# lasgroup/Model-based-policy-optimizers

Hardware: NVIDIA B200
Metric: iCEM model-rollout transitions/sec (pop x horizon x problems x CEM iterations) (higher is better)
Workload: dtype f32

## Files before the change

### model-based-policy-optimizers_b200/csrc/icem_kernels.cuh

```cuda
#pragma once
#include <cuda_runtime.h>

#include "noise.cuh"
#include "pendulum.cuh"
#include "select.cuh"
#include "systems.cuh"

namespace mbpo {

template <int MATH, bool SMALL = false, typename ActFn>
__device__ __forceinline__ float rollout_return_th(const PendulumConsts& pc, float th0, float w0, int H, ActFn act) {
  float acc = 0.0f;
  float th = th0, w = w0;
#pragma unroll 2
  for (int t = 0; t < H; ++t) {
    float r;
    if (MATH == MBPO_MATH_REFERENCE) pendulum_step_ref_th<SMALL>(pc, th, w, act(t), r);
    else pendulum_step_theta<SMALL>(pc, th, w, act(t), r);
    acc = __fadd_rn(acc, r);
  }
  return __fdiv_rn(acc, static_cast<float>(H));
}

template <int MATH, bool SMALL = false, typename ActFn>
__device__ __forceinline__ float rollout_return(const PendulumConsts& pc, float c0, float s0, float w0, int H,
                                                ActFn act) {
  return rollout_return_th<MATH, SMALL>(pc, atan2_bounded(s0, c0), w0, H, act);
}

template <int MATH>
__device__ __forceinline__ void rollout_return2(const PendulumConsts& pc, float th0, float w0, int H,
                                                const float* __restrict__ row_a, const float* __restrict__ row_b,
                                                float& ret_a, float& ret_b) {
  f32x2_t acc = splat2(0.0f), th = splat2(th0), w = splat2(w0);
#pragma unroll 1
  for (int t = 0; t < H; ++t) {
    f32x2_t neg_r;
    if (MATH == MBPO_MATH_REFERENCE) pendulum_step_ref_th2(pc, th, w, pack2(row_a[t], row_b[t]), neg_r);
    else pendulum_step_theta2(pc, th, w, pack2(row_a[t], row_b[t]), neg_r);
    acc = sub2(acc, neg_r);
  }
  float acc_a, acc_b;
  unpack2(acc, acc_a, acc_b);
  ret_a = __fdiv_rn(acc_a, static_cast<float>(H));
  ret_b = __fdiv_rn(acc_b, static_cast<float>(H));
}

__device__ __forceinline__ float summarize_particles(float ret, int P, int summarize) {
  if (summarize == MBPO_SUMMARIZE_MAX || P == 1) return ret;
  float acc = 0.0f;
  for (int p = 0; p < P; ++p) acc = __fadd_rn(acc, ret);
  return __fdiv_rn(acc, static_cast<float>(P));
}

struct PlanArgs {
  int B, N, Np, K, P, S, H;
  int warm_start, summarize;
  float init_std, alpha, one_minus_alpha, u_min, u_max;
  MbpoPendulumParams sys;
  MbpoGeneralSystemParams gsys;
  float scale[MBPO_MAX_FREQ];
  const float* x0;
  const uint32_t* key_in;
  const float* best_seq_in;
  float* best_seq_out;
  float* best_value_out;
  uint32_t* key_out;
  MbpoIcemTrace trace;
  int zero_value_precomputed;
};

constexpr int PLAN_THREADS = 256;

template <int HT>
struct PlanSmem {
  static constexpr int HS = HT | 1;
  static size_t bytes(int N, int Np, int K, int H_rt = 0) {
    const int H = HT ? HT : H_rt;
    const int hs = H | 1;
    size_t words = static_cast<size_t>(N + 1) * hs
                   + (N + Np)
                   + 2 * (N + 1)
                   + 3 * H
                   + 2 * K
                   + select_scratch_words(K, N + Np)
                   + 8
                   + (HT ? 0 : static_cast<size_t>(PLAN_THREADS) * hs);
    return words * 4;
  }
};

template <int HT>
struct PlanCtaSmem {
  float* act;
  uint32_t* skey;
  uint32_t* flat;
  float* mean;
  float* std_;
  float* best_seq;
  int* elite_idx;
  int* sel_idx;
  uint32_t* sel_scratch;
  float* best_value;
  uint32_t* carry;
  uint32_t* state_key;
  float* stage;
  __device__ __forceinline__ PlanCtaSmem(uint32_t* base, int N, int Np, int K, int H_rt = 0) {
    const int H = HT ? HT : H_rt;
    const int HS = H | 1;
    act = reinterpret_cast<float*>(base);
    skey = base + static_cast<size_t>(N + 1) * HS;
    flat = skey + (N + Np);
    mean = reinterpret_cast<float*>(flat + 2 * (N + 1));
    std_ = mean + H;
    best_seq = std_ + H;
    elite_idx = reinterpret_cast<int*>(best_seq + H);
    sel_idx = elite_idx + K;
    sel_scratch = reinterpret_cast<uint32_t*>(sel_idx + K);
    best_value = reinterpret_cast<float*>(sel_scratch + select_scratch_words(K, N + Np));
    carry = reinterpret_cast<uint32_t*>(best_value + 1);
    state_key = carry + 2;
    stage = reinterpret_cast<float*>(state_key + 5);
  }
};

template <int HT, int PRNG, int MATH, int THREADS>
__device__ __forceinline__ void plan_problem(const PlanArgs& a, const PlanCtaSmem<HT>& sm, const PendulumConsts& pc,
                                             const RefitScalars& rs, const float* prev_best, Key2 key_in,
                                             Key2& key_new, float x_th, float x_w, int slot, int slots,
                                             const TwiddleTable* tw = nullptr) {
  const int H = HT ? HT : a.H;
  const int HS = H | 1;
  const int N = a.N, M = a.N + a.Np, K = a.K;
  const int tid = threadIdx.x;
  float* act = sm.act;
  uint32_t* skey = sm.skey;
  uint32_t* flat = sm.flat;
  float* mean = sm.mean;
  float* std_ = sm.std_;
  float* best_seq = sm.best_seq;

  float m0 = 0.0f;
  if (tid < H && a.warm_start) m0 = prev_best[tid + 1 < H ? tid + 1 : H - 1];
  __syncthreads();
  if (tid < H) {
    mean[tid] = m0;
    std_[tid] = a.init_std;
    best_seq[tid] = m0;
  }
  if (tid < HS) act[static_cast<size_t>(N) * HS + tid] = 0.0f;
  if (tid == 0) {
    *sm.best_value = __int_as_float(0xFF800000);
    Key2 k_opt;
    split2<PRNG>(key_in, k_opt, key_new);
    sm.carry[0] = k_opt.k0;
    sm.carry[1] = k_opt.k1;
  }
  __syncthreads();

  for (int it = 0; it < a.S; ++it) {
    const size_t tslot = static_cast<size_t>(it) * slots + slot;
    Key2 ck{sm.carry[0], sm.carry[1]}, sampling_rng, particles_rng;
    split2<PRNG>(ck, sampling_rng, particles_rng);
    if (PRNG == MBPO_PRNG_LEGACY) {
      for (int j = tid; j < N + 1; j += THREADS) {
        uint32_t y0 = static_cast<uint32_t>(j), y1 = static_cast<uint32_t>(N + 1 + j);
        threefry2x32(sampling_rng.k0, sampling_rng.k1, y0, y1);
        flat[j] = y0;
        flat[N + 1 + j] = y1;
      }
    }
    __syncthreads();
    if (tid == 0) {
      Key2 nk;
      if (PRNG == MBPO_PRNG_LEGACY) { nk.k0 = flat[0]; nk.k1 = flat[1]; }
      else nk = split_at<1>(sampling_rng, static_cast<uint32_t>(N + 1), 0u);
      sm.carry[0] = nk.k0; sm.carry[1] = nk.k1;
    }

    const int jobs = (it == 0 && !a.zero_value_precomputed) ? N + 1 : N;
    if (it == 0 && a.zero_value_precomputed && tid == THREADS - 1) {
      const uint32_t zk = total_order_key(a.best_value_out[slot]);
      for (int j = N; j < M; ++j) skey[j] = zk;
    }
    for (int n0 = tid; n0 < jobs; n0 += 2 * THREADS) {
      const int n1 = n0 + THREADS;
#pragma unroll 1
      for (int h = 0; h < 2; ++h) {
        const int n = h ? n1 : n0;
        if (n >= N) continue;
        Key2 skey_n;
        if (PRNG == MBPO_PRNG_LEGACY) { skey_n.k0 = flat[2 * (n + 1)]; skey_n.k1 = flat[2 * (n + 1) + 1]; }
        else skey_n = split_at<1>(sampling_rng, static_cast<uint32_t>(N + 1), static_cast<uint32_t>(n + 1));
        const Key2 dim_key = split1<PRNG>(skey_n);
        float* row = act + static_cast<size_t>(n) * HS;
        auto emit = [&](int t, float y) {
          const float v = __fadd_rn(mean[t], __fmul_rn(y, std_[t]));
          row[t] = fminf(fmaxf(v, a.u_min), a.u_max);
        };
        if constexpr (HT != 0) colored_noise_row<HT, PRNG>(dim_key, a.scale, row, nullptr, emit);
        else colored_noise_row_rt<PRNG>(H, dim_key, a.scale, *tw, sm.stage + static_cast<size_t>(tid) * HS, nullptr, emit);
      }
      const int r0 = n0 < N ? n0 : N, r1 = n1 < N ? n1 : N;
      float ret0, ret1;
      rollout_return2<MATH>(pc, x_th, x_w, H, act + static_cast<size_t>(r0) * HS, act + static_cast<size_t>(r1) * HS,
                            ret0, ret1);
#pragma unroll
      for (int h = 0; h < 2; ++h) {
        const int n = h ? n1 : n0;
        const float val = summarize_particles(h ? ret1 : ret0, a.P, a.summarize);
        if (n < N) {
          skey[n] = total_order_key(val);
          if (a.trace.values) a.trace.values[tslot * M + n] = val;
          if (a.trace.actions) {
            const float* row = act + static_cast<size_t>(n) * HS;
            float* dst = a.trace.actions + (tslot * M + n) * H;
            for (int t = 0; t < H; ++t) dst[t] = row[t];
          }
        } else if (n == N && it == 0) {
          const uint32_t zk = total_order_key(val);
          for (int j = N; j < M; ++j) skey[j] = zk;
        }
      }
    }
    __syncthreads();
    if (a.trace.values || a.trace.actions) {
      const uint32_t zk = skey[N];
      const float zv = __uint_as_float((zk & 0x80000000u) ? (zk & 0x7FFFFFFFu) : ~zk);
      for (int j = N + tid; j < M; j += THREADS) {
        if (a.trace.values) a.trace.values[tslot * M + j] = zv;
        if (a.trace.actions) {
          float* dst = a.trace.actions + (tslot * M + j) * H;
          for (int t = 0; t < H; ++t) dst[t] = 0.0f;
        }
      }
    }

    cta_select_refit<THREADS>(rs, skey, sm.elite_idx, sm.sel_idx, sm.sel_scratch,
                              [&](int i, int d) { return i < N ? act[static_cast<size_t>(i) * HS + d] : 0.0f; },
                              mean, std_, best_seq, sm.best_value);
    if (a.trace.elite_idx)
      for (int e = tid; e < K; e += THREADS) a.trace.elite_idx[tslot * K + e] = sm.elite_idx[e];
    for (int d = tid; d < H; d += THREADS) {
      if (a.trace.mean) a.trace.mean[tslot * H + d] = mean[d];
      if (a.trace.std) a.trace.std[tslot * H + d] = std_[d];
    }
    if (a.trace.best_value && tid == 0) a.trace.best_value[tslot] = *sm.best_value;
    __syncthreads();
  }
}

template <int MATH>
__global__ void zero_row_value_kernel(const MbpoPendulumParams sys, int H, int P, int summarize,
                                      const float* __restrict__ x0, int B, float* __restrict__ out) {
  const int b = blockIdx.x * blockDim.x + threadIdx.x;
  if (b >= B) return;
  const PendulumConsts pc(sys);
  const float ret = rollout_return<MATH, true>(pc, x0[3 * b], x0[3 * b + 1], x0[3 * b + 2], H,
                                               [](int) { return 0.0f; });
  out[b] = summarize_particles(ret, P, summarize);
}

template <int HT, int PRNG, int MATH, int THREADS>
__device__ __forceinline__ void plan_kernel_body(const PlanArgs& a, const TwiddleTable* tw) {
  extern __shared__ __align__(16) uint32_t smem_u32[];
  const int H = HT ? HT : a.H;
  const PlanCtaSmem<HT> sm(smem_u32, a.N, a.Np, a.K, H);
  const int tid = threadIdx.x;
  const PendulumConsts pc(a.sys);
  RefitScalars rs;
  rs.M = a.N + a.Np; rs.K = a.K; rs.D = H; rs.alpha = a.alpha; rs.one_minus_alpha = a.one_minus_alpha;

  for (int b = blockIdx.x; b < a.B; b += gridDim.x) {
    const float x_c = a.x0[3 * b], x_s = a.x0[3 * b + 1], x_w = a.x0[3 * b + 2];
    Key2 k_in{a.key_in[2 * b], a.key_in[2 * b + 1]}, k_new;
    plan_problem<HT, PRNG, MATH, THREADS>(a, sm, pc, rs, a.best_seq_in + static_cast<size_t>(b) * H, k_in, k_new,
                                          atan2_bounded(x_s, x_c), x_w, b, a.B, tw);
    if (tid < H) a.best_seq_out[static_cast<size_t>(b) * H + tid] = sm.best_seq[tid];
    if (tid == 0) {
      a.best_value_out[b] = *sm.best_value;
      a.key_out[2 * b] = k_new.k0;
      a.key_out[2 * b + 1] = k_new.k1;
    }
    __syncthreads();
  }
}

template <int H, int PRNG, int MATH, int THREADS, int MINB>
__global__ void __launch_bounds__(THREADS, MINB) icem_plan_pendulum_kernel(const __grid_constant__ PlanArgs a) {
  plan_kernel_body<H, PRNG, MATH, THREADS>(a, nullptr);
}

template <int PRNG, int MATH>
__global__ void __launch_bounds__(PLAN_THREADS, 1)
    icem_plan_pendulum_rt_kernel(const __grid_constant__ PlanArgs a, const __grid_constant__ TwiddleTable tw) {
  plan_kernel_body<0, PRNG, MATH, PLAN_THREADS>(a, &tw);
}

struct MpcArgs {
  int T;
  float* states_out;
  float* rewards_out;
  float* actions_out;
};

template <int HT, int PRNG, int MATH, int THREADS>
__device__ __forceinline__ void mpc_kernel_body(const PlanArgs& a, const MpcArgs& m, const TwiddleTable* tw) {
  extern __shared__ __align__(16) uint32_t smem_u32[];
  const int H = HT ? HT : a.H;
  const PlanCtaSmem<HT> sm(smem_u32, a.N, a.Np, a.K, H);
  __shared__ float xs[4];
  const int tid = threadIdx.x;
  const PendulumConsts pc(a.sys);
  RefitScalars rs;
  rs.M = a.N + a.Np; rs.K = a.K; rs.D = H; rs.alpha = a.alpha; rs.one_minus_alpha = a.one_minus_alpha;

  for (int b = blockIdx.x; b < a.B; b += gridDim.x) {
    if (tid < H) sm.best_seq[tid] = a.best_seq_in[static_cast<size_t>(b) * H + tid];
    if (tid < 3) xs[tid] = a.x0[3 * b + tid];
    if (tid == 0) { sm.state_key[0] = a.key_in[2 * b]; sm.state_key[1] = a.key_in[2 * b + 1]; }
    __syncthreads();
    for (int t = 0; t < m.T; ++t) {
      const float x_c = xs[0], x_s = xs[1], x_w = xs[2];
      Key2 k_in{sm.state_key[0], sm.state_key[1]}, k_new;
      plan_problem<HT, PRNG, MATH, THREADS>(a, sm, pc, rs, sm.best_seq, k_in, k_new, atan2_bounded(x_s, x_c), x_w, 0,
                                            1, tw);
      if (tid == 0) {
        sm.state_key[0] = k_new.k0; sm.state_key[1] = k_new.k1;
        const float u = sm.best_seq[0];
        float c = x_c, s = x_s, w = x_w, r;
        if (MATH == MBPO_MATH_REFERENCE) {
          pendulum_step_ref(pc, c, s, w, u, r);
        } else {
          float th = atan2_bounded(s, c);
          pendulum_step_theta(pc, th, w, u, r);
          sincos_bounded(th, s, c);
        }
        xs[0] = c; xs[1] = s; xs[2] = w;
        const size_t o = static_cast<size_t>(t) * a.B + b;
        if (m.states_out) { m.states_out[o * 3] = c; m.states_out[o * 3 + 1] = s; m.states_out[o * 3 + 2] = w; }
        if (m.rewards_out) m.rewards_out[o] = r;
        if (m.actions_out) m.actions_out[o] = u;
      }
      __syncthreads();
    }
    if (tid < H) a.best_seq_out[static_cast<size_t>(b) * H + tid] = sm.best_seq[tid];
    if (tid == 0) {
      a.best_value_out ? (void)(a.best_value_out[b] = *sm.best_value) : (void)0;
      a.key_out[2 * b] = sm.state_key[0];
      a.key_out[2 * b + 1] = sm.state_key[1];
    }
    __syncthreads();
  }
}

template <int H, int PRNG, int MATH, int THREADS, int MINB>
__global__ void __launch_bounds__(THREADS, MINB)
    icem_mpc_pendulum_kernel(const __grid_constant__ PlanArgs a, const __grid_constant__ MpcArgs m) {
  mpc_kernel_body<H, PRNG, MATH, THREADS>(a, m, nullptr);
}

template <int PRNG, int MATH>
__global__ void __launch_bounds__(PLAN_THREADS, 1)
    icem_mpc_pendulum_rt_kernel(const __grid_constant__ PlanArgs a, const __grid_constant__ MpcArgs m,
                                const __grid_constant__ TwiddleTable tw) {
  mpc_kernel_body<0, PRNG, MATH, PLAN_THREADS>(a, m, &tw);
}

template <int H, int A>
struct GenPlanSmem {
  static constexpr int RS = (H * A) | 1;
  static size_t bytes(int N, int Np, int K) {
    const size_t words = static_cast<size_t>(N + 1) * RS + (N + Np) + 3 * H * A + 2 * K +
                         select_scratch_words(K, N + Np) + 8;
    return words * 4;
  }
};

template <class Sys, int H, int PRNG>
__global__ void __launch_bounds__(256, 1) icem_plan_general_kernel(const __grid_constant__ PlanArgs a) {
  constexpr int A = Sys::A, X = Sys::X, D = H * A, RS = GenPlanSmem<H, A>::RS, THREADS = 256;
  extern __shared__ __align__(16) uint32_t smem_u32[];
  const int N = a.N, M = a.N + a.Np, K = a.K;
  float* act = reinterpret_cast<float*>(smem_u32);
  uint32_t* skey = smem_u32 + static_cast<size_t>(N + 1) * RS;
  float* mean = reinterpret_cast<float*>(skey + M);
  float* std_ = mean + D;
  float* best_seq = std_ + D;
  int* elite_idx = reinterpret_cast<int*>(best_seq + D);
  int* sel_idx = elite_idx + K;
  uint32_t* scratch = reinterpret_cast<uint32_t*>(sel_idx + K);
  float* best_value = reinterpret_cast<float*>(scratch + select_scratch_words(K, M));
  uint32_t* carry = reinterpret_cast<uint32_t*>(best_value + 1);
  const int tid = threadIdx.x;
  const Sys sys(a.gsys);
  RefitScalars rs;
  rs.M = M; rs.K = K; rs.D = D; rs.alpha = a.alpha; rs.one_minus_alpha = a.one_minus_alpha;
  auto elem = [&](int i, int d) { return i < N ? act[static_cast<size_t>(i) * RS + (d % A) * H + d / A] : 0.0f; };

  for (int b = blockIdx.x; b < a.B; b += gridDim.x) {
    float s0[X];
#pragma unroll
    for (int k = 0; k < X; ++k) s0[k] = a.x0[static_cast<size_t>(b) * X + k];
    const float* prev = a.best_seq_in + static_cast<size_t>(b) * D;
    for (int d = tid; d < D; d += THREADS) {
      float m = 0.0f;
      if (a.warm_start) m = prev[(d + A < D) ? d + A : (D - A + d % A)];
      mean[d] = m;
      std_[d] = a.init_std;
      best_seq[d] = m;
    }
    for (int d = tid; d < RS; d += THREADS) act[static_cast<size_t>(N) * RS + d] = 0.0f;
    Key2 k_new{0u, 0u};
    if (tid == 0) {
      *best_value = __int_as_float(0xFF800000);
      Key2 k_opt;
      split2<PRNG>(Key2{a.key_in[2 * b], a.key_in[2 * b + 1]}, k_opt, k_new);
      carry[0] = k_opt.k0;
      carry[1] = k_opt.k1;
    }
    __syncthreads();
    float zero_value = 0.0f;

    for (int it = 0; it < a.S; ++it) {
      const size_t tslot = static_cast<size_t>(it) * a.B + b;
      Key2 ck{carry[0], carry[1]}, sampling_rng, particles_rng;
      split2<PRNG>(ck, sampling_rng, particles_rng);
      __syncthreads();
      if (tid == 0) {
        const Key2 nk = split_at<PRNG>(sampling_rng, static_cast<uint32_t>(N + 1), 0u);
        carry[0] = nk.k0;
        carry[1] = nk.k1;
      }
      const int jobs = Sys::KEYED ? M : ((it == 0) ? N + 1 : N);
      for (int n = tid; n < jobs; n += THREADS) {
        float* row = act + static_cast<size_t>(n < N ? n : N) * RS;
        if (n < N) {
          const Key2 sk = split_at<PRNG>(sampling_rng, static_cast<uint32_t>(N + 1), static_cast<uint32_t>(n + 1));
#pragma unroll 1
          for (int ad = 0; ad < A; ++ad) {
            const Key2 dk = split_at<PRNG>(sk, static_cast<uint32_t>(A), static_cast<uint32_t>(ad));
            float* dim = row + ad * H;
            colored_noise_row<H, PRNG>(dk, a.scale, dim, nullptr, [&](int t, float y) {
              const float v = __fadd_rn(mean[t * A + ad], __fmul_rn(y, std_[t * A + ad]));
              dim[t] = fminf(fmaxf(v, a.u_min), a.u_max);
            });
          }
        }
        float val;
        auto roll = [&](Key2 key) {
          float s[X];
#pragma unroll
          for (int k = 0; k < X; ++k) s[k] = s0[k];
          float acc = 0.0f;
          for (int t = 0; t < H; ++t) acc = __fadd_rn(acc, sys.template step<PRNG>(s, row + t, H, key));
          return __fdiv_rn(acc, static_cast<float>(H));
        };
        if (!Sys::KEYED) {
          const float ret = roll(Key2{0u, 0u});
          if (a.summarize == MBPO_SUMMARIZE_MAX || a.P == 1) {
            val = ret;
          } else {
            float acc = 0.0f;
            for (int p = 0; p < a.P; ++p) acc = __fadd_rn(acc, ret);
            val = __fdiv_rn(acc, static_cast<float>(a.P));
          }
        } else {
          const Key2 pkey = split_at<PRNG>(particles_rng, static_cast<uint32_t>(M), static_cast<uint32_t>(n));
          float acc = 0.0f, mx = 0.0f;
          for (int p = 0; p < a.P; ++p) {
            const float ret = roll(split_at<PRNG>(pkey, static_cast<uint32_t>(a.P), static_cast<uint32_t>(p)));
            acc = __fadd_rn(acc, ret);
            mx = (p == 0) ? ret : fmaxf(mx, ret);
          }
          val = (a.summarize == MBPO_SUMMARIZE_MAX) ? mx : __fdiv_rn(acc, static_cast<float>(a.P));
        }
        if (n < N || Sys::KEYED) {
          skey[n] = total_order_key(val);
          if (a.trace.values) a.trace.values[tslot * M + n] = val;
        } else {
          zero_value = val;
          for (int j = N; j < M; ++j) skey[j] = total_order_key(val);
        }
        if (a.trace.actions) {
          float* dst = a.trace.actions + (tslot * M + n) * D;
          for (int d = 0; d < D; ++d) dst[d] = (n < N) ? row[(d % A) * H + d / A] : 0.0f;
        }
      }
      __syncthreads();
      if (!Sys::KEYED && (a.trace.values || a.trace.actions)) {
        const float zv = value_of_key(skey[N]);
        for (int j = N + tid; j < M; j += THREADS) {
          if (a.trace.values) a.trace.values[tslot * M + j] = zv;
          if (a.trace.actions && !(j == N && it == 0)) {
            float* dst = a.trace.actions + (tslot * M + j) * D;
            for (int d = 0; d < D; ++d) dst[d] = 0.0f;
          }
        }
      }
      (void)zero_value;
      cta_select_refit<THREADS>(rs, skey, elite_idx, sel_idx, scratch, elem, mean, std_, best_seq, best_value);
      if (a.trace.elite_idx)
        for (int e = tid; e < K; e += THREADS) a.trace.elite_idx[tslot * K + e] = elite_idx[e];
      for (int d = tid; d < D; d += THREADS) {
        if (a.trace.mean) a.trace.mean[tslot * D + d] = mean[d];
        if (a.trace.std) a.trace.std[tslot * D + d] = std_[d];
      }
      if (a.trace.best_value && tid == 0) a.trace.best_value[tslot] = *best_value;
      __syncthreads();
    }
    for (int d = tid; d < D; d += THREADS) a.best_seq_out[static_cast<size_t>(b) * D + d] = best_seq[d];
    if (tid == 0) {
      a.best_value_out[b] = *best_value;
      a.key_out[2 * b] = k_new.k0;
      a.key_out[2 * b + 1] = k_new.k1;
    }
    __syncthreads();
  }
}


struct ScaleTable {
  float v[MBPO_MAX_FREQ];
};

constexpr int STAGED_THREADS = 128;

template <int H, int PRNG>
__global__ void __launch_bounds__(STAGED_THREADS) powerlaw_noise_kernel(const __grid_constant__ ScaleTable tbl, const uint32_t* __restrict__ keys, int M,
                                      float* __restrict__ out, uint32_t* __restrict__ bits_out) {
  __shared__ float stage[STAGED_THREADS][H | 1];
  const int i = blockIdx.x * blockDim.x + threadIdx.x;
  if (i >= M) return;
  Key2 k{keys[2 * i], keys[2 * i + 1]};
  float* row = out + static_cast<size_t>(i) * H;
  colored_noise_row<H, PRNG>(k, tbl.v, stage[threadIdx.x],
                             bits_out ? bits_out + static_cast<size_t>(i) * 2 * NoiseShape<H>::F : nullptr,
                             [&](int t, float y) { row[t] = y; });
}

template <int H, int PRNG>
__global__ void __launch_bounds__(STAGED_THREADS) sample_actions_kernel(const __grid_constant__ ScaleTable tbl, const uint32_t* __restrict__ carry_key,
                                      const float* __restrict__ mean, const float* __restrict__ std_, int N, int Np,
                                      int A, float u_min, float u_max, float* __restrict__ actions,
                                      uint32_t* __restrict__ next_key, uint32_t* __restrict__ particle_keys) {
  __shared__ float stage[STAGED_THREADS][H | 1];
  const int b = blockIdx.y;
  const int M = N + Np;
  const int idx = blockIdx.x * blockDim.x + threadIdx.x;
  if (idx >= M * A) return;
  const int n = idx / A, ad = idx % A;
  Key2 ck{carry_key[2 * b], carry_key[2 * b + 1]}, sampling_rng, particles_rng;
  split2<PRNG>(ck, sampling_rng, particles_rng);
  if (ad == 0 && particle_keys) {
    const Key2 pk = split_at<PRNG>(particles_rng, static_cast<uint32_t>(M), static_cast<uint32_t>(n));
    particle_keys[(static_cast<size_t>(b) * M + n) * 2] = pk.k0;
    particle_keys[(static_cast<size_t>(b) * M + n) * 2 + 1] = pk.k1;
  }
  if (idx == 0) {
    const Key2 nk = split_at<PRNG>(sampling_rng, static_cast<uint32_t>(N + 1), 0u);
    next_key[2 * b] = nk.k0;
    next_key[2 * b + 1] = nk.k1;
  }
  float* row = actions + (static_cast<size_t>(b) * M + n) * H * A + ad;
  if (n >= N) {
    for (int t = 0; t < H; ++t) row[static_cast<size_t>(t) * A] = 0.0f;
    return;
  }
  const Key2 sk = split_at<PRNG>(sampling_rng, static_cast<uint32_t>(N + 1), static_cast<uint32_t>(n + 1));
  const Key2 dk = split_at<PRNG>(sk, static_cast<uint32_t>(A), static_cast<uint32_t>(ad));
  const float* mrow = mean + static_cast<size_t>(b) * H * A + ad;
  const float* srow = std_ + static_cast<size_t>(b) * H * A + ad;
  colored_noise_row<H, PRNG>(dk, tbl.v, stage[threadIdx.x], nullptr, [&](int t, float y) {
    const float v = __fadd_rn(mrow[static_cast<size_t>(t) * A], __fmul_rn(y, srow[static_cast<size_t>(t) * A]));
    row[static_cast<size_t>(t) * A] = fminf(fmaxf(v, u_min), u_max);
  });
}

template <int PRNG>
__global__ void __launch_bounds__(STAGED_THREADS)
    powerlaw_noise_rt_kernel(const __grid_constant__ ScaleTable tbl, const __grid_constant__ TwiddleTable tw, int H,
                             const uint32_t* __restrict__ keys, int M, float* __restrict__ out,
                             uint32_t* __restrict__ bits_out) {
  extern __shared__ __align__(16) float stage_rt[];
  const int i = blockIdx.x * blockDim.x + threadIdx.x;
  if (i >= M) return;
  Key2 k{keys[2 * i], keys[2 * i + 1]};
  float* row = out + static_cast<size_t>(i) * H;
  colored_noise_row_rt<PRNG>(H, k, tbl.v, tw, stage_rt + static_cast<size_t>(threadIdx.x) * (H | 1),
                             bits_out ? bits_out + static_cast<size_t>(i) * 2 * (H / 2 + 1) : nullptr,
                             [&](int t, float y) { row[t] = y; });
}

template <int PRNG>
__global__ void __launch_bounds__(STAGED_THREADS)
    sample_actions_rt_kernel(const __grid_constant__ ScaleTable tbl, const __grid_constant__ TwiddleTable tw, int H,
                             const uint32_t* __restrict__ carry_key, const float* __restrict__ mean,
                             const float* __restrict__ std_, int N, int Np, int A, float u_min, float u_max,
                             float* __restrict__ actions, uint32_t* __restrict__ next_key,
                             uint32_t* __restrict__ particle_keys) {
  extern __shared__ __align__(16) float stage_rt[];
  const int b = blockIdx.y;
  const int M = N + Np;
  const int idx = blockIdx.x * blockDim.x + threadIdx.x;
  if (idx >= M * A) return;
  const int n = idx / A, ad = idx % A;
  Key2 ck{carry_key[2 * b], carry_key[2 * b + 1]}, sampling_rng, particles_rng;
  split2<PRNG>(ck, sampling_rng, particles_rng);
  if (ad == 0 && particle_keys) {
    const Key2 pk = split_at<PRNG>(particles_rng, static_cast<uint32_t>(M), static_cast<uint32_t>(n));
    particle_keys[(static_cast<size_t>(b) * M + n) * 2] = pk.k0;
    particle_keys[(static_cast<size_t>(b) * M + n) * 2 + 1] = pk.k1;
  }
  if (idx == 0) {
    const Key2 nk = split_at<PRNG>(sampling_rng, static_cast<uint32_t>(N + 1), 0u);
    next_key[2 * b] = nk.k0;
    next_key[2 * b + 1] = nk.k1;
  }
  float* row = actions + (static_cast<size_t>(b) * M + n) * H * A + ad;
  if (n >= N) {
    for (int t = 0; t < H; ++t) row[static_cast<size_t>(t) * A] = 0.0f;
    return;
  }
  const Key2 sk = split_at<PRNG>(sampling_rng, static_cast<uint32_t>(N + 1), static_cast<uint32_t>(n + 1));
  const Key2 dk = split_at<PRNG>(sk, static_cast<uint32_t>(A), static_cast<uint32_t>(ad));
  const float* mrow = mean + static_cast<size_t>(b) * H * A + ad;
  const float* srow = std_ + static_cast<size_t>(b) * H * A + ad;
  colored_noise_row_rt<PRNG>(H, dk, tbl.v, tw, stage_rt + static_cast<size_t>(threadIdx.x) * (H | 1), nullptr,
                             [&](int t, float y) {
    const float v = __fadd_rn(mrow[static_cast<size_t>(t) * A], __fmul_rn(y, srow[static_cast<size_t>(t) * A]));
    row[static_cast<size_t>(t) * A] = fminf(fmaxf(v, u_min), u_max);
  });
}

}
```

### model-based-policy-optimizers_b200/csrc/select.cuh

```cuda
#pragma once
#include "mathx.cuh"

namespace mbpo {

#ifdef MBPO_CLUSTER_CLOCKS
__device__ long long g_select_clocks[16];
#define MBPO_SEL_CLK(i) do { if (threadIdx.x == 0 && blockIdx.x == 0) g_select_clocks[i] = clock64(); } while (0)
#else
#define MBPO_SEL_CLK(i) do {} while (0)
#endif

struct RefitScalars {
  int M;
  int K;
  int D;
  float alpha;
  float one_minus_alpha;
};

constexpr int SELECT_HIST_WORDS = 288;
constexpr int SELECT_HEAD_WORDS = SELECT_HIST_WORDS + 8;
__host__ __device__ constexpr int select_scratch_words(int K, int M) { return SELECT_HEAD_WORDS + K + M; }
__device__ __forceinline__ uint32_t select_hist_slot(uint32_t bin) { return bin + (bin >> 3); }

template <int THREADS>
__device__ __forceinline__ int cta_threads() { return THREADS ? THREADS : static_cast<int>(blockDim.x); }

template <int THREADS>
__device__ __forceinline__ void cta_select(const RefitScalars rs, const uint32_t* keys, int* elite_idx, int* sel_idx,
                                           uint32_t* scratch) {
  const int NT = cta_threads<THREADS>();
  const unsigned full = 0xFFFFFFFFu;
  const int tid = threadIdx.x;
  const int lane = tid & 31;
  const int M = rs.M, K = rs.K;
  uint32_t* hist = scratch;
  uint32_t* misc = scratch + SELECT_HIST_WORDS;
  uint32_t* sel_key = scratch + SELECT_HEAD_WORDS;
  int* cand = reinterpret_cast<int*>(scratch + SELECT_HEAD_WORDS + K);

  MBPO_SEL_CLK(0);
  for (int i = tid; i < SELECT_HEAD_WORDS; i += NT) scratch[i] = (i == SELECT_HIST_WORDS + 1) ? 0xFFFFFFFFu : 0u;
  __syncthreads();
  {
    uint32_t o = 0u, a = 0xFFFFFFFFu;
    for (int i = tid; i < M; i += NT) {
      const uint32_t k = keys[i];
      o |= k;
      a &= k;
    }
    o = __reduce_or_sync(full, o);
    a = __reduce_and_sync(full, a);
    if (lane == 0) {
      atomicOr(&misc[0], o);
      atomicAnd(&misc[1], a);
    }
  }
  __syncthreads();
  const uint32_t diff = misc[0] ^ misc[1];
  const int hb = 31 - __clz(diff | 1u);
  const int shift = hb > 7 ? hb - 7 : 0;

  MBPO_SEL_CLK(1);
  for (int i = tid; i < M; i += NT) atomicAdd(&hist[select_hist_slot((keys[i] >> shift) & 255u)], 1u);
  __syncthreads();

  MBPO_SEL_CLK(2);
  int bb, n_above;
  {
    uint32_t h8[8];
    uint32_t s = 0;
#pragma unroll
    for (int j = 0; j < 8; ++j) {
      h8[j] = hist[lane * 9 + j];
      s += h8[j];
    }
    uint32_t suf = s;
#pragma unroll
    for (int off = 1; off < 32; off <<= 1) {
      const uint32_t v = __shfl_down_sync(full, suf, off);
      if (lane + off < 32) suf += v;
    }
    const unsigned ok = __ballot_sync(full, static_cast<int>(suf) >= K);
    const int L = 31 - __clz(ok);
    int my_bb = 0, my_above = 0;
    if (lane == L) {
      uint32_t above = suf - s;
      my_bb = lane * 8;
#pragma unroll
      for (int j = 7; j >= 0; --j) {
        if (static_cast<int>(above + h8[j]) >= K) {
          my_bb = lane * 8 + j;
          break;
        }
        above += h8[j];
      }
      my_above = static_cast<int>(above);
    }
    bb = __shfl_sync(full, my_bb, L);
    n_above = __shfl_sync(full, my_above, L);
  }

  MBPO_SEL_CLK(3);
  for (int base = 0; base < M; base += NT) {
    const int i = base + tid;
    uint32_t k = 0u;
    int d = -1;
    if (i < M) {
      k = keys[i];
      d = static_cast<int>((k >> shift) & 255u);
    }
    const unsigned above = __ballot_sync(full, d > bb);
    const unsigned inside = __ballot_sync(full, d == bb);
    uint32_t pos_a = 0u, pos_c = 0u;
    if (lane == 0) {
      if (above) pos_a = atomicAdd(&misc[2], static_cast<uint32_t>(__popc(above)));
      if (inside) pos_c = atomicAdd(&misc[3], static_cast<uint32_t>(__popc(inside)));
    }
    pos_a = __shfl_sync(full, pos_a, 0);
    pos_c = __shfl_sync(full, pos_c, 0);
    const unsigned lt = (1u << lane) - 1u;
    if (d > bb) {
      const uint32_t pos = pos_a + static_cast<uint32_t>(__popc(above & lt));
      sel_idx[pos] = i;
      sel_key[pos] = k;
    } else if (d == bb) {
      cand[pos_c + static_cast<uint32_t>(__popc(inside & lt))] = i;
    }
  }
  __syncthreads();

  MBPO_SEL_CLK(4);
  const int nc = static_cast<int>(misc[3]);
  for (int base = 0; base < 4 * (n_above + nc); base += NT) {
    const int w = base + tid;
    const int item = w >> 2, g = w & 3;
    int larger = 0, ie = 0;
    if (item < n_above) {
      ie = sel_idx[item];
      const uint32_t ke = sel_key[item];
      for (int f = g; f < n_above; f += 4) {
        const int jf = sel_idx[f];
        const uint32_t kf = sel_key[f];
        larger += (kf > ke || (kf == ke && jf > ie)) ? 1 : 0;
      }
    } else if (item < n_above + nc) {
      ie = cand[item - n_above];
      const uint32_t ke = keys[ie];
      larger = (g == 0) ? n_above : 0;
      for (int f = g; f < nc; f += 4) {
        const int jf = cand[f];
        const uint32_t kf = keys[jf];
        larger += (kf > ke || (kf == ke && jf > ie)) ? 1 : 0;
      }
    }
    larger += __shfl_xor_sync(full, larger, 1);
    larger += __shfl_xor_sync(full, larger, 2);
    if (item < n_above + nc && g == 0 && larger < K) elite_idx[K - 1 - larger] = ie;
  }
  __syncthreads();
  MBPO_SEL_CLK(5);
  MBPO_SEL_CLK(6);

}

__device__ __forceinline__ float value_of_key(uint32_t k) {
  return __uint_as_float((k & 0x80000000u) ? (k & 0x7FFFFFFFu) : ~k);
}

template <typename EliteFn>
__device__ __forceinline__ void refit_column(const RefitScalars& rs, EliteFn elite, int d, float m_old, float s_old,
                                             float& m_new, float& s_new) {
  const int K = rs.K;
  const float kf = static_cast<float>(K);
  float acc = 0.0f;
#pragma unroll 5
  for (int e = 0; e < K; ++e) acc = __fadd_rn(acc, elite(e, d));
  const float emean = __fdiv_rn(acc, kf);
  acc = 0.0f;
#pragma unroll 5
  for (int e = 0; e < K; ++e) {
    const float dl = __fsub_rn(elite(e, d), emean);
    acc = __fadd_rn(acc, __fmul_rn(dl, dl));
  }
  const float evar = __fdiv_rn(acc, kf);
  m_new = __fadd_rn(__fmul_rn(m_old, rs.alpha), __fmul_rn(rs.one_minus_alpha, emean));
  const float var = __fadd_rn(__fmul_rn(__fmul_rn(s_old, s_old), rs.alpha), __fmul_rn(rs.one_minus_alpha, evar));
  s_new = __fsqrt_rn(var);
}

template <int THREADS, typename EliteFn>
__device__ __forceinline__ void cta_refit(const RefitScalars rs, float best_elite, EliteFn elite, float* mean,
                                          float* std_, float* best_seq, float* best_value) {
  const int NT = cta_threads<THREADS>();
  const int tid = threadIdx.x;
  const int K = rs.K;
  const bool take = (*best_value <= best_elite);
  __syncthreads();
  for (int d = tid; d < rs.D; d += NT) {
    float m_new, s_new;
    refit_column(rs, elite, d, mean[d], std_[d], m_new, s_new);
    mean[d] = m_new;
    std_[d] = s_new;
    if (take) best_seq[d] = elite(K - 1, d);
  }
  if (tid == 0 && take) *best_value = best_elite;
  __syncthreads();
}

template <int THREADS, typename RowFn>
__device__ __forceinline__ void cta_select_refit(const RefitScalars rs, const uint32_t* keys, int* elite_idx,
                                                 int* sel_idx, uint32_t* scratch, RowFn row, float* mean,
                                                 float* std_, float* best_seq, float* best_value) {
  cta_select<THREADS>(rs, keys, elite_idx, sel_idx, scratch);
  const float best_elite = value_of_key(keys[elite_idx[rs.K - 1]]);
  cta_refit<THREADS>(rs, best_elite, [&](int e, int d) { return row(elite_idx[e], d); }, mean, std_, best_seq,
                     best_value);
}

}
```

Baseline: 144.0 billion.

## Overlap next-iteration key schedule with refit and fold key OR/AND during rollout

Moves per-iteration PRNG key derivation (threefry/split to per-row dim keys) into a schedule that a subset of threads (those beyond the refit's H columns) runs during the refit phase of the previous CEM iteration, using a named barrier and double-buffered sampling keys. The select's key OR/AND reduction is folded into the rollout loop, so cta_select skips its reset and key scan passes, and one trailing __syncthreads is removed. This cuts serial per-iteration work and barriers, at the cost of more complex synchronization, with a risk of races on the shared scratch and flat buffers.

```diff
diff --git a/model-based-policy-optimizers_b200/csrc/icem_kernels.cuh b/model-based-policy-optimizers_b200/csrc/icem_kernels.cuh
--- a/model-based-policy-optimizers_b200/csrc/icem_kernels.cuh
+++ b/model-based-policy-optimizers_b200/csrc/icem_kernels.cuh
@@ -102,7 +102,7 @@
   int* sel_idx;
   uint32_t* sel_scratch;
   float* best_value;
-  uint32_t* carry;
+  uint32_t* srng;
   uint32_t* state_key;
   float* stage;
   __device__ __forceinline__ PlanCtaSmem(uint32_t* base, int N, int Np, int K, int H_rt = 0) {
@@ -118,11 +118,43 @@
     sel_idx = elite_idx + K;
     sel_scratch = reinterpret_cast<uint32_t*>(sel_idx + K);
     best_value = reinterpret_cast<float*>(sel_scratch + select_scratch_words(K, N + Np));
-    carry = reinterpret_cast<uint32_t*>(best_value + 1);
-    state_key = carry + 2;
-    stage = reinterpret_cast<float*>(state_key + 5);
+    srng = reinterpret_cast<uint32_t*>(best_value + 1);
+    state_key = srng + 4;
+    stage = reinterpret_cast<float*>(state_key + 3);
   }
 };
+
+template <int PRNG, typename Bar>
+__device__ __forceinline__ void plan_key_schedule(int N, uint32_t* flat, const uint32_t* srng_cur, uint32_t* srng_next,
+                                                  int t, int gn, Bar bar) {
+  const Key2 srng{srng_cur[0], srng_cur[1]};
+  if (PRNG == MBPO_PRNG_LEGACY) {
+    for (int j = t; j < N + 1; j += gn) {
+      uint32_t y0 = static_cast<uint32_t>(j), y1 = static_cast<uint32_t>(N + 1 + j);
+      threefry2x32(srng.k0, srng.k1, y0, y1);
+      flat[j] = y0;
+      flat[N + 1 + j] = y1;
+    }
+    bar();
+  }
+  for (int n = t; n < N; n += gn) {
+    uint32_t* w = flat + 2 * (n + 1);
+    Key2 rk;
+    if (PRNG == MBPO_PRNG_LEGACY) rk = Key2{w[0], w[1]};
+    else rk = split_at<1>(srng, static_cast<uint32_t>(N + 1), static_cast<uint32_t>(n + 1));
+    const Key2 dk = split1<PRNG>(rk);
+    w[0] = dk.k0;
+    w[1] = dk.k1;
+  }
+  if (t == gn - 1) {
+    Key2 ck, next, particles_rng;
+    if (PRNG == MBPO_PRNG_LEGACY) ck = Key2{flat[0], flat[1]};
+    else ck = split_at<1>(srng, static_cast<uint32_t>(N + 1), 0u);
+    split2<PRNG>(ck, next, particles_rng);
+    srng_next[0] = next.k0;
+    srng_next[1] = next.k1;
+  }
+}
 
 template <int HT, int PRNG, int MATH, int THREADS>
 __device__ __forceinline__ void plan_problem(const PlanArgs& a, const PlanCtaSmem<HT>& sm, const PendulumConsts& pc,
@@ -136,6 +168,7 @@
   float* act = sm.act;
   uint32_t* skey = sm.skey;
   uint32_t* flat = sm.flat;
+  uint32_t* scratch = sm.sel_scratch;
   float* mean = sm.mean;
   float* std_ = sm.std_;
   float* best_seq = sm.best_seq;
@@ -149,39 +182,33 @@
     best_seq[tid] = m0;
   }
   if (tid < HS) act[static_cast<size_t>(N) * HS + tid] = 0.0f;
+  select_reset(scratch, tid, THREADS);
   if (tid == 0) {
     *sm.best_value = __int_as_float(0xFF800000);
-    Key2 k_opt;
+    Key2 k_opt, sampling_rng, particles_rng;
     split2<PRNG>(key_in, k_opt, key_new);
-    sm.carry[0] = k_opt.k0;
-    sm.carry[1] = k_opt.k1;
+    split2<PRNG>(k_opt, sampling_rng, particles_rng);
+    sm.srng[0] = sampling_rng.k0;
+    sm.srng[1] = sampling_rng.k1;
   }
   __syncthreads();
+  plan_key_schedule<PRNG>(N, flat, sm.srng, sm.srng + 2, tid, THREADS, [] { __syncthreads(); });
+  __syncthreads();
+  const int g0 = (H + 31) & ~31;
+  const int gn = THREADS - g0;
 
   for (int it = 0; it < a.S; ++it) {
     const size_t tslot = static_cast<size_t>(it) * slots + slot;
-    Key2 ck{sm.carry[0], sm.carry[1]}, sampling_rng, particles_rng;
-    split2<PRNG>(ck, sampling_rng, particles_rng);
-    if (PRNG == MBPO_PRNG_LEGACY) {
-      for (int j = tid; j < N + 1; j += THREADS) {
-        uint32_t y0 = static_cast<uint32_t>(j), y1 = static_cast<uint32_t>(N + 1 + j);
-        threefry2x32(sampling_rng.k0, sampling_rng.k1, y0, y1);
-        flat[j] = y0;
-        flat[N + 1 + j] = y1;
-      }
-    }
-    __syncthreads();
-    if (tid == 0) {
-      Key2 nk;
-      if (PRNG == MBPO_PRNG_LEGACY) { nk.k0 = flat[0]; nk.k1 = flat[1]; }
-      else nk = split_at<1>(sampling_rng, static_cast<uint32_t>(N + 1), 0u);
-      sm.carry[0] = nk.k0; sm.carry[1] = nk.k1;
-    }
-
+    if (it == a.S - 1) MBPO_SEL_CLK(11);
+
+    uint32_t ko = 0u, ka = 0xFFFFFFFFu;
     const int jobs = (it == 0 && !a.zero_value_precomputed) ? N + 1 : N;
-    if (it == 0 && a.zero_value_precomputed && tid == THREADS - 1) {
-      const uint32_t zk = total_order_key(a.best_value_out[slot]);
-      for (int j = N; j < M; ++j) skey[j] = zk;
+    if (M > N && tid == THREADS - 1 && (it > 0 || a.zero_value_precomputed)) {
+      const uint32_t zk = it > 0 ? skey[N] : total_order_key(a.best_value_out[slot]);
+      if (it == 0)
+        for (int j = N; j < M; ++j) skey[j] = zk;
+      ko = zk;
+      ka = zk;
     }
     for (int n0 = tid; n0 < jobs; n0 += 2 * THREADS) {
       const int n1 = n0 + THREADS;
@@ -189,10 +216,7 @@
       for (int h = 0; h < 2; ++h) {
         const int n = h ? n1 : n0;
         if (n >= N) continue;
-        Key2 skey_n;
-        if (PRNG == MBPO_PRNG_LEGACY) { skey_n.k0 = flat[2 * (n + 1)]; skey_n.k1 = flat[2 * (n + 1) + 1]; }
-        else skey_n = split_at<1>(sampling_rng, static_cast<uint32_t>(N + 1), static_cast<uint32_t>(n + 1));
-        const Key2 dim_key = split1<PRNG>(skey_n);
+        const Key2 dim_key{flat[2 * (n + 1)], flat[2 * (n + 1) + 1]};
         float* row = act + static_cast<size_t>(n) * HS;
         auto emit = [&](int t, float y) {
           const float v = __fadd_rn(mean[t], __fmul_rn(y, std_[t]));
@@ -210,7 +234,10 @@
         const int n = h ? n1 : n0;
         const float val = summarize_particles(h ? ret1 : ret0, a.P, a.summarize);
         if (n < N) {
-          skey[n] = total_order_key(val);
+          const uint32_t k = total_order_key(val);
+          skey[n] = k;
+          ko |= k;
+          ka &= k;
           if (a.trace.values) a.trace.values[tslot * M + n] = val;
           if (a.trace.actions) {
             const float* row = act + static_cast<size_t>(n) * HS;
@@ -220,10 +247,16 @@
         } else if (n == N && it == 0) {
           const uint32_t zk = total_order_key(val);
           for (int j = N; j < M; ++j) skey[j] = zk;
-        }
-      }
-    }
+          if (M > N) {
+            ko |= zk;
+            ka &= zk;
+          }
+        }
+      }
+    }
+    select_fold_keys(scratch, ko, ka);
     __syncthreads();
+    if (it == a.S - 2) MBPO_SEL_CLK(7);
     if (a.trace.values || a.trace.actions) {
       const uint32_t zk = skey[N];
       const float zv = __uint_as_float((zk & 0x80000000u) ? (zk & 0x7FFFFFFFu) : ~zk);
@@ -236,9 +269,20 @@
       }
     }
 
-    cta_select_refit<THREADS>(rs, skey, sm.elite_idx, sm.sel_idx, sm.sel_scratch,
-                              [&](int i, int d) { return i < N ? act[static_cast<size_t>(i) * HS + d] : 0.0f; },
-                              mean, std_, best_seq, sm.best_value);
+    const bool next = it + 1 < a.S;
+    cta_select_refit<THREADS, true>(
+        rs, skey, sm.elite_idx, sm.sel_idx, scratch,
+        [&](int i, int d) { return i < N ? act[static_cast<size_t>(i) * HS + d] : 0.0f; }, mean, std_, best_seq,
+        sm.best_value, [&] {
+          if (next && tid >= g0) {
+            if (it == a.S - 2) MBPO_SEL_CLK_AT(9, THREADS - 1);
+            select_reset(scratch, tid - g0, gn);
+            plan_key_schedule<PRNG>(N, flat, sm.srng + 2 * ((it + 1) & 1), sm.srng + 2 * (it & 1), tid - g0, gn,
+                                    [gn] { asm volatile("bar.sync 1, %0;" ::"r"(gn) : "memory"); });
+            if (it == a.S - 2) MBPO_SEL_CLK_AT(10, THREADS - 1);
+          }
+        });
+    if (it == a.S - 2) MBPO_SEL_CLK(8);
     if (a.trace.elite_idx)
       for (int e = tid; e < K; e += THREADS) a.trace.elite_idx[tslot * K + e] = sm.elite_idx[e];
     for (int d = tid; d < H; d += THREADS) {
@@ -246,7 +290,6 @@
       if (a.trace.std) a.trace.std[tslot * H + d] = std_[d];
     }
     if (a.trace.best_value && tid == 0) a.trace.best_value[tslot] = *sm.best_value;
-    __syncthreads();
   }
 }
 
diff --git a/model-based-policy-optimizers_b200/csrc/select.cuh b/model-based-policy-optimizers_b200/csrc/select.cuh
--- a/model-based-policy-optimizers_b200/csrc/select.cuh
+++ b/model-based-policy-optimizers_b200/csrc/select.cuh
@@ -5,10 +5,11 @@
 
 #ifdef MBPO_CLUSTER_CLOCKS
 __device__ long long g_select_clocks[16];
-#define MBPO_SEL_CLK(i) do { if (threadIdx.x == 0 && blockIdx.x == 0) g_select_clocks[i] = clock64(); } while (0)
+#define MBPO_SEL_CLK_AT(i, t) do { if (threadIdx.x == (t) && blockIdx.x == 0) g_select_clocks[i] = clock64(); } while (0)
 #else
-#define MBPO_SEL_CLK(i) do {} while (0)
+#define MBPO_SEL_CLK_AT(i, t) do {} while (0)
 #endif
+#define MBPO_SEL_CLK(i) MBPO_SEL_CLK_AT(i, 0)
 
 struct RefitScalars {
   int M;
@@ -23,10 +24,23 @@
 __host__ __device__ constexpr int select_scratch_words(int K, int M) { return SELECT_HEAD_WORDS + K + M; }
 __device__ __forceinline__ uint32_t select_hist_slot(uint32_t bin) { return bin + (bin >> 3); }
 
+__device__ __forceinline__ void select_reset(uint32_t* scratch, int t, int nt) {
+  for (int i = t; i < SELECT_HEAD_WORDS; i += nt) scratch[i] = (i == SELECT_HIST_WORDS + 1) ? 0xFFFFFFFFu : 0u;
+}
+
+__device__ __forceinline__ void select_fold_keys(uint32_t* scratch, uint32_t o, uint32_t a) {
+  o = __reduce_or_sync(0xFFFFFFFFu, o);
+  a = __reduce_and_sync(0xFFFFFFFFu, a);
+  if ((threadIdx.x & 31) == 0) {
+    atomicOr(&scratch[SELECT_HIST_WORDS], o);
+    atomicAnd(&scratch[SELECT_HIST_WORDS + 1], a);
+  }
+}
+
 template <int THREADS>
 __device__ __forceinline__ int cta_threads() { return THREADS ? THREADS : static_cast<int>(blockDim.x); }
 
-template <int THREADS>
+template <int THREADS, bool KEYS_FOLDED = false>
 __device__ __forceinline__ void cta_select(const RefitScalars rs, const uint32_t* keys, int* elite_idx, int* sel_idx,
                                            uint32_t* scratch) {
   const int NT = cta_threads<THREADS>();
@@ -40,23 +54,18 @@
   int* cand = reinterpret_cast<int*>(scratch + SELECT_HEAD_WORDS + K);
 
   MBPO_SEL_CLK(0);
-  for (int i = tid; i < SELECT_HEAD_WORDS; i += NT) scratch[i] = (i == SELECT_HIST_WORDS + 1) ? 0xFFFFFFFFu : 0u;
-  __syncthreads();
-  {
+  if (!KEYS_FOLDED) {
+    select_reset(scratch, tid, NT);
+    __syncthreads();
     uint32_t o = 0u, a = 0xFFFFFFFFu;
     for (int i = tid; i < M; i += NT) {
       const uint32_t k = keys[i];
       o |= k;
       a &= k;
     }
-    o = __reduce_or_sync(full, o);
-    a = __reduce_and_sync(full, a);
-    if (lane == 0) {
-      atomicOr(&misc[0], o);
-      atomicAnd(&misc[1], a);
-    }
-  }
-  __syncthreads();
+    select_fold_keys(scratch, o, a);
+    __syncthreads();
+  }
   const uint32_t diff = misc[0] ^ misc[1];
   const int hb = 31 - __clz(diff | 1u);
   const int shift = hb > 7 ? hb - 7 : 0;
@@ -189,9 +198,13 @@
   s_new = __fsqrt_rn(var);
 }
 
-template <int THREADS, typename EliteFn>
+struct NoOverlap {
+  __device__ __forceinline__ void operator()() const {}
+};
+
+template <int THREADS, typename EliteFn, typename Under = NoOverlap>
 __device__ __forceinline__ void cta_refit(const RefitScalars rs, float best_elite, EliteFn elite, float* mean,
-                                          float* std_, float* best_seq, float* best_value) {
+                                          float* std_, float* best_seq, float* best_value, Under under = {}) {
   const int NT = cta_threads<THREADS>();
   const int tid = threadIdx.x;
   const int K = rs.K;
@@ -205,17 +218,18 @@
     if (take) best_seq[d] = elite(K - 1, d);
   }
   if (tid == 0 && take) *best_value = best_elite;
-  __syncthreads();
-}
-
-template <int THREADS, typename RowFn>
+  under();
+  __syncthreads();
+}
+
+template <int THREADS, bool KEYS_FOLDED = false, typename RowFn, typename Under = NoOverlap>
 __device__ __forceinline__ void cta_select_refit(const RefitScalars rs, const uint32_t* keys, int* elite_idx,
                                                  int* sel_idx, uint32_t* scratch, RowFn row, float* mean,
-                                                 float* std_, float* best_seq, float* best_value) {
-  cta_select<THREADS>(rs, keys, elite_idx, sel_idx, scratch);
+                                                 float* std_, float* best_seq, float* best_value, Under under = {}) {
+  cta_select<THREADS, KEYS_FOLDED>(rs, keys, elite_idx, sel_idx, scratch);
   const float best_elite = value_of_key(keys[elite_idx[rs.K - 1]]);
   cta_refit<THREADS>(rs, best_elite, [&](int e, int d) { return row(elite_idx[e], d); }, mean, std_, best_seq,
-                     best_value);
-}
-
-}
+                     best_value, under);
+}
+
+}
```

Result: faster. 147.2 billion, median of 6 (+2.2%).
